# uibk-uncover/ws-unet

Measured on AMD Instinct MI355X. Metric: 512x512 grayscale images/sec (UNet predict), higher is better.
Workload: dtype f16 MFMA on the f16 halves + ONE block-scaled fp4 (e2m1) MFMA per tap pair for both residual cross terms (per-pixel / per-(co, tap) E8M0 scales), fp32 accumulate; planar storage

## Files before the change

### ws_unet_amd/csrc/conv3x3_q.hip

```cpp
#include "wsu_device.h"
#include <cstdlib>

namespace {

constexpr int TW = 32, TH = 16, IW = TW + 2, IH = TH + 2;
constexpr int NPIX = IW * IH;
constexpr int PLANE = NPIX * 16;
constexpr int IN_SEG = (NPIX + 63) / 64;
constexpr int S_LDS = IN_SEG * 256;
constexpr int IN_SLOT = 3 * PLANE + S_LDS;
constexpr int W_GRAN = 9 * 3 * WSU_COB * 16;
constexpr int W_SLOT = W_GRAN + 1024;
constexpr int NIN = 3, NWS = 2;
constexpr int W_BASE = NIN * IN_SLOT;
constexpr int LDS_EXTRA = W_BASE + NWS * W_SLOT;
constexpr int LDS_TOTAL = LDS_EXTRA + 1024 * 4 + 4 * 64 * 4 + 16;
static_assert(LDS_TOTAL <= 160 * 1024 && W_SLOT % 1024 == 0, "LDS budget");
constexpr int NLOAD = 4;
constexpr int W_PIECES = W_SLOT / 1024;
constexpr unsigned OOB = 0xFFFFFFF0u;
constexpr int IN_SLOT_H = 2 * PLANE;
constexpr int W_SLOT_H = 9 * 2 * WSU_COB * 16;
template <int FMT> struct QGeo {
    static_assert(FMT == WSU_PLANAR_Q || FMT == WSU_PLANAR_H, "conv3x3_q_kernel formats: Q and H");
// ... 234 lines not shown
        switch (wv - NWAVE) {
            case 0: q_loader<FMT, 0>(a, smem, lane, lw, G, J); break;
            case 1: q_loader<FMT, 1>(a, smem, lane, lw, G, J); break;
            case 2: q_loader<FMT, 2>(a, smem, lane, lw, G, J); break;
            default: q_loader<FMT, 3>(a, smem, lane, lw, G, J); break;
        }
        return;
    }

    Tile cur = tile_of(a, lw);
    constexpr int MH = MSPLIT ? 1 : 2;
    constexpr bool PIPE = RQ == 4 && !H;
    constexpr bool EPO = !MSPLIT && HC == 0 && RQ != 4;
    f32x16 acc[2][4];
    int kt = 0, j = 0;
    unsigned q_in_off = 0, q_w_off = 0;
    const char* ldsA = smem;
    const char* ldsB = smem;
    int hh_q = hh;
    auto begin_step = [&]() __attribute__((always_inline)) {
        __builtin_amdgcn_s_barrier();
        asm volatile("" ::: "memory");
        q_in_off = (unsigned)(j % NIN) * Gm::in_slot; q_w_off = Gm::w_base + (unsigned)(j % NWS) * Gm::w_slot;
        ldsA = smem + q_w_off + (cur.mh * 32 + l31) * 16;
        ldsB = smem + q_in_off + ((RQ * wv) * IW + l31) * 16;
        hh_q = hh;
        asm volatile("" : "+v"(hh_q));
    };
    auto zero_acc = [&]() __attribute__((always_inline)) {
#pragma unroll
        for (int m = 0; m < MH; ++m)
#pragma unroll
            for (int q = 0; q < RQ; ++q)
#pragma unroll
                for (int r = 0; r < 16; ++r) acc[m][q][r] = 0.f;
    };
    auto main_term = [&](auto tap_c, auto ms_c) __attribute__((always_inline)) {
        constexpr int tap = decltype(tap_c)::value, dy = tap / 3, dx = tap % 3;
        constexpr int ms = decltype(ms_c)::value, ML = ms < 0 ? 0 : ms, MU = ms < 0 ? MH : ms + 1;
        u32x4 ah[2], bh[4];
_Pragma("unroll")
        for (int m = ML; m < MU; ++m) ah[m] = *reinterpret_cast<const u32x4*>(ldsA + ((tap * Gm::w_planes + hh) * 64 + m * 32) * 16);
_Pragma("unroll")
        for (int q = 0; q < RQ; ++q) bh[q] = *reinterpret_cast<const u32x4*>(ldsB + hh * PLANE + ((q + dy) * IW + dx) * 16);
_Pragma("unroll")
        for (int m = ML; m < MU; ++m)
_Pragma("unroll")
            for (int q = 0; q < RQ; ++q) wsu_mfma_f16(ah[m], bh[q], acc[m][q]);
    };
    auto cross_q4 = [&](auto tp_c, auto ms_c) __attribute__((always_inline)) {
        constexpr int tp = decltype(tp_c)::value;
        constexpr int ms = decltype(ms_c)::value, ML = ms < 0 ? 0 : ms, MU = ms < 0 ? MH : ms + 1;
        constexpr int t0 = 2 * tp, t1 = (2 * tp + 1 < 9) ? 2 * tp + 1 : 2 * tp;
        constexpr bool single = 2 * tp + 1 >= 9;
        const int tap = hh_q ? t1 : t0;
        const int pixoff = (tap / 3) * IW + tap % 3;
        u32x4 a4[2], b4[4]; int sa[2], sb[4];
        typedef __attribute__((address_space(3))) const unsigned char lds_cuchar;
        typedef __attribute__((address_space(3))) const int lds_cint;
        typedef __attribute__((address_space(3))) const u32x4 lds_cu32x4;
        lds_char* L = (lds_char*)smem;
        const unsigned wbase = q_w_off + (unsigned)(cur.mh * 32 + l31) * 16u + (unsigned)((tap * 3 + 2) * 64) * 16u;
        const unsigned sabase = q_w_off + W_GRAN + (unsigned)(tap * 64 + cur.mh * 32 + l31);
        const unsigned pix = (unsigned)((RQ * wv) * IW + l31 + pixoff);
_Pragma("unroll")
        for (int m = ML; m < MU; ++m) {
            a4[m] = *(lds_cu32x4*)(L + wbase + m * 32 * 16);
            sa[m] = *(lds_cuchar*)(L + sabase + m * 32);
        }
_Pragma("unroll")
        for (int q = 0; q < RQ; ++q) {
            b4[q] = *(lds_cu32x4*)(L + q_in_off + 2 * PLANE + (pix + q * IW) * 16u);
            sb[q] = *(lds_cint*)(L + q_in_off + 3 * PLANE + (pix + q * IW) * 4u);
        }
        if (single && hh_q) {
            const u32x4 z = mk_u4(0, 0, 0, 0);
_Pragma("unroll")
            for (int m = ML; m < MU; ++m) a4[m] = z;
_Pragma("unroll")
            for (int q = 0; q < RQ; ++q) b4[q] = z;
        }
_Pragma("unroll")
        for (int m = ML; m < MU; ++m)
_Pragma("unroll")
            for (int q = 0; q < RQ; ++q) wsu_mfma_q4(a4[m], b4[q], sa[m], sb[q], acc[m][q]);
    };
    auto units_range = [&](auto ms_c, auto lo_c, auto hi_c) __attribute__((always_inline)) {
        constexpr int lo = decltype(lo_c)::value, hi = decltype(hi_c)::value;
        if constexpr (EPO) asm volatile("" : "+v"(hh_q));
        WSU_STATIC_FOR(hi - lo, i, {
            constexpr int tp = lo + i;
            if constexpr (!H) cross_q4(std::integral_constant<int, tp>{}, ms_c);
            main_term(std::integral_constant<int, 2 * tp>{}, ms_c);
            if constexpr (2 * tp + 1 < 9) main_term(std::integral_constant<int, 2 * tp + 1>{}, ms_c);
        });
    };
    constexpr std::integral_constant<int, -1> all_m{};
    struct Frag { u32x4 a[2]; u32x4 b[4]; int sa[2]; int sb[4]; };
    auto load_unit = [&](auto u_c, Frag& f) __attribute__((always_inline)) {
        constexpr int u = decltype(u_c)::value, tp = u / 3, k = u % 3;
        typedef __attribute__((address_space(3))) const unsigned char lds_cuchar;
        typedef __attribute__((address_space(3))) const int lds_cint;
        typedef __attribute__((address_space(3))) const u32x4 lds_cu32x4;
        lds_char* L = (lds_char*)smem;
        if constexpr (k == 0) {
            constexpr int t0 = 2 * tp, t1 = (2 * tp + 1 < 9) ? 2 * tp + 1 : 2 * tp;
            const int tap = hh_q ? t1 : t0;
            const int pixoff = (tap / 3) * IW + tap % 3;
            const unsigned wbase = q_w_off + (unsigned)(cur.mh * 32 + l31) * 16u + (unsigned)((tap * 3 + 2) * 64) * 16u;
            const unsigned sabase = q_w_off + W_GRAN + (unsigned)(tap * 64 + cur.mh * 32 + l31);
            const unsigned pix = (unsigned)((RQ * wv) * IW + l31 + pixoff);
_Pragma("unroll")
            for (int m = 0; m < MH; ++m) {
                f.a[m] = *(lds_cu32x4*)(L + wbase + m * 32 * 16);
                f.sa[m] = *(lds_cuchar*)(L + sabase + m * 32);
            }
_Pragma("unroll")
            for (int q = 0; q < RQ; ++q) {
                f.b[q] = *(lds_cu32x4*)(L + q_in_off + 2 * PLANE + (pix + q * IW) * 16u);
                f.sb[q] = *(lds_cint*)(L + q_in_off + 3 * PLANE + (pix + q * IW) * 4u);
            }
        } else {
            constexpr int tap = 2 * tp + k - 1, dy = tap / 3, dx = tap % 3;
            const unsigned abase = q_w_off + (unsigned)((cur.mh * 32 + l31) * 16) + (unsigned)(hh_q * 64 * 16);
            const unsigned bbase = q_in_off + (unsigned)(((RQ * wv) * IW + l31) * 16) + (unsigned)(hh_q * PLANE);
_Pragma("unroll")
            for (int m = 0; m < MH; ++m) f.a[m] = *(lds_cu32x4*)(L + abase + ((tap * 3) * 64 + m * 32) * 16);
_Pragma("unroll")
            for (int q = 0; q < RQ; ++q) f.b[q] = *(lds_cu32x4*)(L + bbase + ((q + dy) * IW + dx) * 16);
        }
    };
    auto mma_unit = [&](auto u_c, Frag& f) __attribute__((always_inline)) {
        constexpr int u = decltype(u_c)::value, tp = u / 3, k = u % 3;
        if constexpr (k == 0) {
            if (2 * tp + 1 >= 9 && hh_q) {
                const u32x4 z = mk_u4(0, 0, 0, 0);
_Pragma("unroll")
                for (int m = 0; m < MH; ++m) f.a[m] = z;
_Pragma("unroll")
                for (int q = 0; q < RQ; ++q) f.b[q] = z;
            }
_Pragma("unroll")
            for (int m = 0; m < MH; ++m)
_Pragma("unroll")
                for (int q = 0; q < RQ; ++q) wsu_mfma_q4(f.a[m], f.b[q], f.sa[m], f.sb[q], acc[m][q]);
        } else {
_Pragma("unroll")
            for (int m = 0; m < MH; ++m)
_Pragma("unroll")
                for (int q = 0; q < RQ; ++q) wsu_mfma_f16(f.a[m], f.b[q], acc[m][q]);
        }
    };
    auto units_pipelined = [&]() __attribute__((always_inline)) {
        constexpr int NU = 14;
        Frag fr[2];
        load_unit(std::integral_constant<int, 0>{}, fr[0]);
        WSU_STATIC_FOR(NU, u, {
            if constexpr (u + 1 < NU) load_unit(std::integral_constant<int, u + 1>{}, fr[(u + 1) % 2]);
            __builtin_amdgcn_sched_barrier(0);
            mma_unit(u_c, fr[u % 2]);
            __builtin_amdgcn_sched_barrier(0);
        });
    };
    auto units_all = [&](auto ms_c) __attribute__((always_inline)) {
        if constexpr (PIPE && decltype(ms_c)::value < 0) { units_pipelined(); return; }
        units_range(ms_c, std::integral_constant<int, 0>{}, std::integral_constant<int, 5>{});
    };

    auto finish_tile = [&]() __attribute__((always_inline)) {
        int l31 = l31_k, hh = hh_k;
        asm volatile("" : "+v"(l31), "+v"(hh));
        const int col = cur.x0 + l31;
        const unsigned hw16 = (unsigned)(a.h * a.w) * 16u;
        const int nco = a.cout >> 4;
        float hz[4][HC > 0 ? HC : 1];
        float vmax = 0.f;
        const float relu_floor = a.relu ? 0.f : -__builtin_inff();
#pragma unroll
        for (int q = 0; q < RQ; ++q)
#pragma unroll
            for (int o = 0; o < (HC > 0 ? HC : 1); ++o) hz[q][o] = 0.f;
// ... 26 lines not shown
        };
        auto store_one_a = [&](const f32x4& X, const f32x4& Y, char* base, unsigned plane_bytes, unsigned off, bool ok, bool have) __attribute__((always_inline)) {
            uint32_t xh0, xh1, xlo, yh0, yh1, ylo;
            wsu_split4_f16r8(X, WSU_F8_XLO_DIV, xh0, xh1, xlo);
            wsu_split4_f16r8(Y, WSU_F8_XLO_DIV, yh0, yh1, ylo);
            wsu_swap32(xh0, yh0); wsu_swap32(xh1, yh1);
            uint32_t xlp = xlo, ylp = ylo;
            wsu_swap32(xlo, xlp); wsu_swap32(ylo, ylp);
            const auto rs = __builtin_amdgcn_make_buffer_rsrc(base, 0, have ? (int)(3u * plane_bytes) : 0, 0x00020000);
            __builtin_amdgcn_raw_buffer_store_b128(mk_u4(xh0, xh1, yh0, yh1), rs, (int)(ok ? off + (hh ? plane_bytes : 0u) : OOB), 0, 0);
            __builtin_amdgcn_raw_buffer_store_b128(mk_u4(xlo, xlp, ylo, ylp), rs, (int)((ok && !hh) ? off + 2u * plane_bytes : OOB), 0, 0);
        };
        auto epi_m = [&](auto m_c, auto&& hook) __attribute__((always_inline)) {
            constexpr int m = decltype(m_c)::value;
            constexpr int NH = RQ / 2;
            auto piece = [&](auto cp_c) __attribute__((always_inline)) {
                constexpr int cp = decltype(cp_c)::value;
                const int oc = cur.cb * 4 + (m + cur.mh) * 2 + cp;
                const int co0 = oc * 16 + 4 * hh;
                const bool have_y = a.y != nullptr;
                f32x4 px[2], py[2];
                WSU_STATIC_FOR(RQ / 2, rp, {
                    hook(std::integral_constant<int, NH * cp + rp>{});
                    f32x4 vx[2], vy[2];
                    const f32x4 bx = *reinterpret_cast<const f32x4*>(s_bias + co0), by = *reinterpret_cast<const f32x4*>(s_bias + co0 + 8);
_Pragma("unroll")
                    for (int u = 0; u < 2; ++u) {
_Pragma("unroll")
                        for (int e = 0; e < 4; ++e) {
                            const float x = fmaxf(acc[m][2 * rp + u][8 * cp + e] + bx[e], relu_floor), y = fmaxf(acc[m][2 * rp + u][8 * cp + 4 + e] + by[e], relu_floor);
// ... 47 lines not shown
                    const int gy0 = (cur.y0 >> 1) + (RQ / 2) * wv, gx = (cur.x0 >> 1) + (l31 >> 1);
                    const bool okx = !(l31 & 1) && gx < wp2;
                    const unsigned php16 = (unsigned)(hp * wp2) * 16u;
                    if constexpr (H) {
                        char* base = a.ypool + ((size_t)cur.n * nco + oc) * (2u * php16);
#pragma unroll
                        for (int rp = 0; rp < RQ / 2; ++rp)
                            store_one_h(px[rp], py[rp], base, php16, (unsigned)((gy0 + rp) * wp2 + gx) * 16u, okx && gy0 + rp < hp, true);
                    } else if constexpr (FQ) {
                        const unsigned cbp = (unsigned)wsu_q_chunk_bytes(hp, wp2);
                        const int ptx = (wp2 + 31) >> 5;
                        char* base = a.ypool + ((size_t)cur.n * nco + oc) * cbp;
                        if constexpr (RQ == 4) {
                            store_pair_q(px[0], py[0], px[1], py[1], base, cbp, php16, (unsigned)(gy0 * wp2 + gx) * 16u, (unsigned)((gy0 + 1) * wp2 + gx) * 16u,
                                         wsu_q_soff(gy0, gx, ptx), wsu_q_soff(gy0 + 1, gx, ptx), okx && gy0 < hp, okx && gy0 + 1 < hp, true);
                        } else {
                            store_one_q(px[0], py[0], base, cbp, php16, (unsigned)(gy0 * wp2 + gx) * 16u, wsu_q_soff(gy0, gx, ptx), okx && gy0 < hp, true);
                        }
                    } else {
                        char* base = a.ypool + (((size_t)cur.n * nco + oc) * 3) * php16;
#pragma unroll
                        for (int rp = 0; rp < RQ / 2; ++rp)
                            store_one_a(px[rp], py[rp], base, php16, (unsigned)((gy0 + rp) * wp2 + gx) * 16u, okx && gy0 + rp < hp, true);
                    }
                }
            };
            piece(std::integral_constant<int, 0>{});
            piece(std::integral_constant<int, 1>{});
        };
        auto nothing = [](auto) __attribute__((always_inline)) {};
        if constexpr (EPO) {
            constexpr int NHT = 2 * (RQ / 2);
            epi_m(std::integral_constant<int, 0>{}, [&](auto h_c) __attribute__((always_inline)) {
                constexpr int h = decltype(h_c)::value;
                constexpr int lo = 5 * h / NHT, hi = 5 * (h + 1) / NHT;
                if constexpr (hi > lo) units_range(std::integral_constant<int, 1>{}, std::integral_constant<int, lo>{}, std::integral_constant<int, hi>{});
            });
            epi_m(std::integral_constant<int, 1>{}, nothing);
        } else {
            WSU_STATIC_FOR(MH, m, { (void)m; epi_m(m_c, nothing); });
        }
        if constexpr (HEAD) {
            const size_t hw = (size_t)a.h * a.w;
#pragma unroll
            for (int q = 0; q < RQ; ++q) {
                const int row = cur.y0 + RQ * wv + q;
#pragma unroll
                for (int o = 0; o < HC; ++o)
                    if (o < a.head_cout) {
                        uint32_t mine = __builtin_bit_cast(uint32_t, hz[q][o]), other = mine;
                        wsu_swap32(mine, other);
// ... 1 lines not shown
                        if (!hh && row < a.h && col < a.w) {
                            const size_t plane = ((size_t)cur.n * a.head_cout + o) * hw;
                            const uint32_t off = (uint32_t)(row * a.w + col);
                            if (a.head_logit) (a.head_logit + plane)[off] = z;
                            (a.head_out + plane)[off] = 1.f / (1.f + expf(-z));
                        }
                    }
            }
        }
        if (a.range_flag && (a.y || POOL) && __builtin_amdgcn_ballot_w64(!(vmax <= (H ? WSU_F16_RANGE : WSU_F8_RANGE))) != 0 && lane == 0)
            atomicOr(a.range_flag, 1u);
        ++kt;
        if (j + 1 < J) cur = tile_of(a, lw + kt * G);
    };
    for (int t = 0; t < K; ++t) {
        zero_acc();
        for (int cc = 1; cc < a.nch; ++cc) { begin_step(); units_all(all_m); ++j; }
        begin_step();
        if constexpr (EPO) units_all(std::integral_constant<int, 0>{});
        else units_all(all_m);
        __builtin_amdgcn_sched_barrier(0);
        finish_tile();
        ++j;
    }
}

__global__ void pack_conv3x3_f4_kernel(const float* __restrict__ w, char* __restrict__ dst, int cin, int cout) {
    const int nch = cin / 16;
    const long long total = (long long)(cout / WSU_COB) * nch * 9 * WSU_COB;
    for (long long d = (long long)blockIdx.x * blockDim.x + threadIdx.x; d < total; d += (long long)gridDim.x * blockDim.x) {
        long long t = d;
        const int co = (int)(t % WSU_COB); t /= WSU_COB;
        const int tap = (int)(t % 9); t /= 9;
        const int c = (int)(t % nch); const int cb = (int)(t / nch);
        float v[16], r[16];
// ... 274 lines not shown
```

### ws_unet_amd/csrc/conv3x3_qu.hip

```cpp
#include "wsu_device.h"

namespace {

constexpr int TW = 32, TH = 16;
constexpr int CW = 17, CH = 9, CPIX = CW * CH;
constexpr int NPIX_S = 4 * CPIX;
constexpr int PLANE_S = NPIX_S * 16;
constexpr int SEG_S = (NPIX_S + 63) / 64;
constexpr int IN_S = 3 * PLANE_S + SEG_S * 256;
constexpr int LP = 33, LH = TH / 2 + 2, LW_ = TW / 2 + 2;
constexpr int NPIX_L = LP * LH;
constexpr int PLANE_L = NPIX_L * 16;
constexpr int SEG_L = (NPIX_L + 63) / 64;
constexpr int IN_L = 3 * PLANE_L + SEG_L * 256;
constexpr int W_GRAN_S = 9 * 3 * WSU_COB * 16;
constexpr int W_S = W_GRAN_S + 1024;
constexpr int W_UNITS_L = 8;
constexpr int W_GRAN_L = W_UNITS_L * 3 * WSU_COB * 16;
constexpr int W_L = W_GRAN_L + 1024;
constexpr int PIECES_S = W_S / 1024, PIECES_L = W_L / 1024;
constexpr int REGION = 80640;
constexpr int OFF_SW = IN_S, OFF_LIN = W_L, OFF_LW1 = W_L + IN_L;
constexpr int LDS_BIAS = 2 * REGION;
constexpr int MAX_COUT = 512;
// ... 195 lines not shown
    const int cls = wv & 3, py = cls >> 1, px = cls & 1, rh = wv >> 2;
    const int l31 = lane & 31, hh = lane >> 5;
    const int lrow = l31 >> 4, lcol = lrow ? ((l31 + 15) & 15) : l31;
    const unsigned laneS = (unsigned)(((4 * rh + lrow) * CW + lcol) * 16), laneL = (unsigned)(((4 * rh + lrow) * LP + lcol) * 16);
    constexpr unsigned QS = 2 * CW * 16, QL = 2 * LP * 16;
    Tile cur = tile_of(a, lw);
    f32x16 acc[2][2];
    unsigned region = 0;
    unsigned in_off = 0, w_off = 0;
    auto next_region = [&]() __attribute__((always_inline)) { const unsigned r = region; region ^= (unsigned)REGION; return r; };
    int hh_q = hh;
    typedef __attribute__((address_space(3))) const unsigned char lds_cuchar;
    typedef __attribute__((address_space(3))) const int lds_cint;
    typedef __attribute__((address_space(3))) const u32x4 lds_cu32x4;
    lds_char* L = (lds_char*)smem;
    auto sync_step = [&]() __attribute__((always_inline)) {
        __builtin_amdgcn_s_barrier();
        asm volatile("" ::: "memory");
        hh_q = hh;
        asm volatile("" : "+v"(hh_q));
    };
    auto tap_s = [&](int ky, int kx) __attribute__((always_inline)) {
        return (unsigned)(((((py + ky) & 1) * 2 + ((px + kx) & 1)) * CPIX + ((py + ky) >> 1) * CW + ((px + kx) >> 1)) * 16);
    };
    auto skip_units = [&]() __attribute__((always_inline)) {
        WSU_STATIC_FOR(5, tp, {
            constexpr int t0 = 2 * tp, t1 = (2 * tp + 1 < 9) ? 2 * tp + 1 : 2 * tp;
            if constexpr (!H) {
                const unsigned tapo = hh_q ? tap_s(t1 / 3, t1 % 3) : tap_s(t0 / 3, t0 % 3);
                const int tap = hh_q ? t1 : t0;
                u32x4 a4[2], b4[2]; int sa[2], sb[2];
                const unsigned wb = w_off + (unsigned)((tap * 3 + 2) * 64 + l31) * 16u, sab = w_off + W_GRAN_S + (unsigned)(tap * 64 + l31);
                const unsigned pb = tapo + laneS;
_Pragma("unroll")
                for (int m = 0; m < 2; ++m) { a4[m] = *(lds_cu32x4*)(L + wb + m * 512); sa[m] = *(lds_cuchar*)(L + sab + m * 32); }
_Pragma("unroll")
                for (int q = 0; q < 2; ++q) {
                    b4[q] = *(lds_cu32x4*)(L + in_off + 2 * PLANE_S + pb + q * QS);
                    sb[q] = *(lds_cint*)(L + in_off + 3 * PLANE_S + ((pb + q * QS) >> 2));
                }
                if (2 * tp + 1 >= 9 && hh_q) {
                    const u32x4 z = mk_u4(0, 0, 0, 0);
                    a4[0] = z; a4[1] = z; b4[0] = z; b4[1] = z;
                }
_Pragma("unroll")
                for (int m = 0; m < 2; ++m)
_Pragma("unroll")
                    for (int q = 0; q < 2; ++q) wsu_mfma_q4(a4[m], b4[q], sa[m], sb[q], acc[m][q]);
            }
            WSU_STATIC_FOR((2 * tp + 1 < 9 ? 2 : 1), k, {
                constexpr int tap = 2 * tp + k;
                u32x4 ah[2], bh[2];
                const unsigned wb = w_off + (unsigned)((tap * WPL) * 64 + l31) * 16u + (unsigned)hh * 1024u;
                const unsigned pb = in_off + (unsigned)hh * PLANE_S + tap_s(tap / 3, tap % 3) + laneS;
_Pragma("unroll")
                for (int m = 0; m < 2; ++m) ah[m] = *(lds_cu32x4*)(L + wb + m * 512);
_Pragma("unroll")
                for (int q = 0; q < 2; ++q) bh[q] = *(lds_cu32x4*)(L + pb + q * QS);
_Pragma("unroll")
                for (int m = 0; m < 2; ++m)
_Pragma("unroll")
                    for (int q = 0; q < 2; ++q) wsu_mfma_f16(ah[m], bh[q], acc[m][q]);
            });
        });
    };
    auto low_units = [&](int dy) __attribute__((always_inline)) {
        const unsigned rowo = (unsigned)(((py + dy) * LP + px) * 16);
        if constexpr (!H) {
            const int u = cls * 2 + hh_q;
            u32x4 a4[2], b4[2]; int sa[2], sb[2];
            const unsigned wb = w_off + (unsigned)((u * 3 + 2) * 64 + l31) * 16u, sab = w_off + W_GRAN_L + (unsigned)(u * 64 + l31);
            const unsigned pb = rowo + (unsigned)hh_q * 16u + laneL;
_Pragma("unroll")
            for (int m = 0; m < 2; ++m) { a4[m] = *(lds_cu32x4*)(L + wb + m * 512); sa[m] = *(lds_cuchar*)(L + sab + m * 32); }
_Pragma("unroll")
            for (int q = 0; q < 2; ++q) {
                b4[q] = *(lds_cu32x4*)(L + in_off + 2 * PLANE_L + pb + q * QL);
                sb[q] = *(lds_cint*)(L + in_off + 3 * PLANE_L + ((pb + q * QL) >> 2));
            }
_Pragma("unroll")
            for (int m = 0; m < 2; ++m)
_Pragma("unroll")
                for (int q = 0; q < 2; ++q) wsu_mfma_q4(a4[m], b4[q], sa[m], sb[q], acc[m][q]);
        }
        WSU_STATIC_FOR(2, dx, {
            u32x4 ah[2], bh[2];
            const unsigned wb = w_off + (unsigned)(((cls * 2 + dx) * WPL) * 64 + l31) * 16u + (unsigned)hh * 1024u;
            const unsigned pb = in_off + (unsigned)hh * PLANE_L + rowo + dx * 16u + laneL;
_Pragma("unroll")
            for (int m = 0; m < 2; ++m) ah[m] = *(lds_cu32x4*)(L + wb + m * 512);
_Pragma("unroll")
            for (int q = 0; q < 2; ++q) bh[q] = *(lds_cu32x4*)(L + pb + q * QL);
_Pragma("unroll")
            for (int m = 0; m < 2; ++m)
_Pragma("unroll")
                for (int q = 0; q < 2; ++q) wsu_mfma_f16(ah[m], bh[q], acc[m][q]);
        });
    };

    auto finish_tile = [&]() __attribute__((always_inline)) {
        int l31o = l31, hho = hh, lro = lrow, lco = lcol;
        asm volatile("" : "+v"(l31o), "+v"(hho), "+v"(lro), "+v"(lco));
        const unsigned hw16 = (unsigned)(a.h * a.w) * 16u;
        const unsigned cbytes = (unsigned)wsu_q_chunk_bytes(a.h, a.w);
        const int nco = a.cout >> 4;
        const int X = cur.x0 + 2 * lco + px;
        const int Y0 = cur.y0 + 2 * (4 * rh + lro) + py, Y1 = Y0 + 4;
// ... 30 lines not shown
                const u32x4 qg = wsu_q4_pair(dh0, dr0, dh1, dr1);
                char* base = a.y + ((size_t)cur.n * nco + oc) * cbytes;
                const auto rs = __builtin_amdgcn_make_buffer_rsrc(base, 0, (int)cbytes, 0x00020000);
                const unsigned hp = hho ? hw16 : 0u;
                __builtin_amdgcn_raw_buffer_store_b128(g0, rs, (int)(ok0 ? off0 + hp : OOB), 0, 0);
                __builtin_amdgcn_raw_buffer_store_b128(g1, rs, (int)(ok1 ? off1 + hp : OOB), 0, 0);
                const bool okm = hho ? ok1 : ok0;
                __builtin_amdgcn_raw_buffer_store_b128(qg, rs, (int)(okm ? (hho ? off1 : off0) + 2u * hw16 : OOB), 0, 0);
                __builtin_amdgcn_raw_buffer_store_b8((unsigned char)(hho ? sb1 : sb0), rs, (int)(okm ? 3u * hw16 + (hho ? so1 : so0) : OOB), 0, 0);
            });
        });
        if (a.range_flag && __builtin_amdgcn_ballot_w64(!(vmax <= (H ? WSU_F16_RANGE : WSU_F8_RANGE))) != 0 && lane == 0) atomicOr(a.range_flag, 1u);
    };

    for (int t = 0; t < K; ++t) {
#pragma unroll
        for (int m = 0; m < 2; ++m)
#pragma unroll
            for (int q = 0; q < 2; ++q)
#pragma unroll
                for (int r = 0; r < 16; ++r) acc[m][q][r] = 0.f;
        for (int c = 0; c < a.nchS; ++c) {
            sync_step();
            const unsigned r = next_region();
            in_off = r; w_off = r + OFF_SW;
            skip_units();
        }
        for (int c = 0; c < a.nchL; ++c) {
            sync_step();
            const unsigned r = next_region();
            in_off = r + OFF_LIN;
            w_off = r;
            low_units(0);
            w_off = r + OFF_LW1;
            low_units(1);
        }
        finish_tile();
        if (t + 1 < K) cur = tile_of(a, lw + (t + 1) * G);
    }
}

template <int FMT>
__global__ void pack_up_low_kernel(const float* __restrict__ w3, const float* __restrict__ wt, char* __restrict__ dst, float* __restrict__ wc_dense,
                                   int cup, int c2, int cl, int cout) {
    const int nchL = cl / 16, ctot = cup + c2;
    const long long total = (long long)(cout / WSU_COB) * nchL * 2 * W_UNITS_L * WSU_COB;
    for (long long d = (long long)blockIdx.x * blockDim.x + threadIdx.x; d < total; d += (long long)gridDim.x * blockDim.x) {
        long long t = d;
        const int co = (int)(t % WSU_COB); t /= WSU_COB;
        const int u = (int)(t % W_UNITS_L); t /= W_UNITS_L;
// ... 166 lines not shown
```

### ws_unet_amd/csrc/wsu_device.h

```cpp
#pragma once
#include <hip/hip_runtime.h>
#include <stdint.h>
#include <type_traits>
#include "../../include/wsu.h"

typedef __attribute__((ext_vector_type(8))) __bf16 bf16x8;
typedef __attribute__((ext_vector_type(16))) float f32x16;
typedef __attribute__((ext_vector_type(4))) float f32x4;
typedef __attribute__((ext_vector_type(4))) uint32_t u32x4;
typedef __attribute__((ext_vector_type(2))) uint32_t u32x2;
__host__ __device__ __forceinline__ u32x4 mk_u4(uint32_t a, uint32_t b, uint32_t c, uint32_t d) { u32x4 v = {a, b, c, d}; return v; }
__host__ __device__ __forceinline__ u32x2 mk_u2(uint32_t a, uint32_t b) { u32x2 v = {a, b}; return v; }
__host__ __device__ __forceinline__ f32x4 mk_f4(float a, float b, float c, float d) { f32x4 v = {a, b, c, d}; return v; }

void wsu_set_error(const char* fmt, ...);
int wsu_check_launch(const char* what);
#define WSU_REQUIRE(cond, ...)            \
    do {                                  \
        if (!(cond)) {                    \
            wsu_set_error(__VA_ARGS__);   \
            return WSU_ERR_ARG;           \
        }                                 \
    } while (0)
#define WSU_INTERNAL extern "C" __attribute__((visibility("hidden")))
// ... 214 lines not shown
    const int e = wsu_q4_block_exp(wsu_f16x16_max_abs_bits(h0, h1));
    const float sc = wsu_pow2f(e), scr = wsu_pow2f(e - 11);
    sb = (uint32_t)(e + 127);
    uint32_t q2 = 0, q3 = 0;
    q2 = __builtin_amdgcn_cvt_scalef32_pk_fp4_f32(q2, r[0], r[1], scr, 0); q2 = __builtin_amdgcn_cvt_scalef32_pk_fp4_f32(q2, r[2], r[3], scr, 1);
    q2 = __builtin_amdgcn_cvt_scalef32_pk_fp4_f32(q2, r[4], r[5], scr, 2); q2 = __builtin_amdgcn_cvt_scalef32_pk_fp4_f32(q2, r[6], r[7], scr, 3);
    q3 = __builtin_amdgcn_cvt_scalef32_pk_fp4_f32(q3, r[8], r[9], scr, 0); q3 = __builtin_amdgcn_cvt_scalef32_pk_fp4_f32(q3, r[10], r[11], scr, 1);
    q3 = __builtin_amdgcn_cvt_scalef32_pk_fp4_f32(q3, r[12], r[13], scr, 2); q3 = __builtin_amdgcn_cvt_scalef32_pk_fp4_f32(q3, r[14], r[15], scr, 3);
    q = mk_u4(wsu_f16x8_to_fp4(h0, sc), wsu_f16x8_to_fp4(h1, sc), q2, q3);
}
__device__ __forceinline__ void wsu_mfma_q4(const u32x4& a, const u32x4& b, int scale_a, int scale_b, f32x16& acc) {
    const i32x8 av = {(int)a.x, (int)a.y, (int)a.z, (int)a.w, 0, 0, 0, 0}, bv = {(int)b.x, (int)b.y, (int)b.z, (int)b.w, 0, 0, 0, 0};
    acc = __builtin_amdgcn_mfma_scale_f32_32x32x64_f8f6f4(av, bv, acc, 4, 4, 0, scale_a, 0, scale_b);
}

__device__ __forceinline__ u32x2 wsu_f16x8_to_fp8_grad(const u32x4& h) {
    const _Float16 m = (_Float16)112.f;
    const f16x8 lim = {m, m, m, m, m, m, m, m};
    const f16x8 c = __builtin_elementwise_max(__builtin_elementwise_min(__builtin_bit_cast(f16x8, h), lim), -lim);
    i16x2 lo = {0, 0}, hi = {0, 0};
    lo = __builtin_amdgcn_cvt_scalef32_pk_fp8_f16(lo, __builtin_shufflevector(c, c, 0, 1), WSU_F8_G_DIV, false);
    lo = __builtin_amdgcn_cvt_scalef32_pk_fp8_f16(lo, __builtin_shufflevector(c, c, 2, 3), WSU_F8_G_DIV, true);
    hi = __builtin_amdgcn_cvt_scalef32_pk_fp8_f16(hi, __builtin_shufflevector(c, c, 4, 5), WSU_F8_G_DIV, false);
    hi = __builtin_amdgcn_cvt_scalef32_pk_fp8_f16(hi, __builtin_shufflevector(c, c, 6, 7), WSU_F8_G_DIV, true);
    return mk_u2(__builtin_bit_cast(uint32_t, lo), __builtin_bit_cast(uint32_t, hi));
}
__device__ __forceinline__ void wsu_mfma_f16(const u32x4& a, const u32x4& b, f32x16& acc) {
    acc = __builtin_amdgcn_mfma_f32_32x32x16_f16(__builtin_bit_cast(f16x8, a), __builtin_bit_cast(f16x8, b), acc, 0, 0, 0);
}
__device__ __forceinline__ void wsu_mfma_f8x2(const u32x4& a_blk0, const u32x4& a_blk1, const u32x4& b_blk0, const u32x4& b_blk1,
                                              int scale_a, int scale_b, f32x16& acc) {
    i32x8 a = {(int)a_blk0.x, (int)a_blk0.y, (int)a_blk0.z, (int)a_blk0.w, (int)a_blk1.x, (int)a_blk1.y, (int)a_blk1.z, (int)a_blk1.w};
    i32x8 b = {(int)b_blk0.x, (int)b_blk0.y, (int)b_blk0.z, (int)b_blk0.w, (int)b_blk1.x, (int)b_blk1.y, (int)b_blk1.z, (int)b_blk1.w};
    acc = __builtin_amdgcn_mfma_scale_f32_32x32x64_f8f6f4(a, b, acc, 0, 0, 0, scale_a, 0, scale_b);
}

__device__ __forceinline__ float wsu_bf16_to_f32(uint16_t v) { return __builtin_bit_cast(float, (uint32_t)v << 16); }

template <int MODE>
__device__ __forceinline__ void wsu_mfma_step(const u32x4& a, const u32x4& b, f32x16& acc) {
    if constexpr (MODE == WSU_MODE_F32) {
        const f32x4 af = __builtin_bit_cast(f32x4, a), bf = __builtin_bit_cast(f32x4, b);
        acc = __builtin_amdgcn_mfma_f32_32x32x2f32(af[0], bf[0], acc, 0, 0, 0);
// ... 23 lines not shown
```

Baseline: 3703.

## Precompute LDS addresses before barrier and fold accumulator zeroing into first MFMA

Computes LDS slot offsets incrementally and hoists per-step base addresses (including the first tap-pair cross-term addresses) ahead of the workgroup barrier, so address arithmetic overlaps the barrier wait instead of following it. The first MFMA of each tile now uses a zero-accumulator variant, which removes the explicit zeroing of the accumulator registers. In the odd-RQ epilogue, two single-channel stores are paired across lanes into one wider store. This adds code complexity and more live VGPRs for the precomputed addresses, which may raise register pressure.

After: 3788 (median of 6 runs). +2.3%, better.

```diff
diff --git a/ws_unet_amd/csrc/conv3x3_q.hip b/ws_unet_amd/csrc/conv3x3_q.hip
--- a/ws_unet_amd/csrc/conv3x3_q.hip
+++ b/ws_unet_amd/csrc/conv3x3_q.hip
@@ -272,18 +272,38 @@
     constexpr bool EPO = !MSPLIT && HC == 0 && RQ != 4;
     f32x16 acc[2][4];
     int kt = 0, j = 0;
-    unsigned q_in_off = 0, q_w_off = 0;
-    const char* ldsA = smem;
-    const char* ldsB = smem;
+    unsigned q_in_off = 0, q_w_off = Gm::w_base;
+    unsigned nx_in = 0, nx_w = Gm::w_base;
+    unsigned a_off = 0, b_off = 0, hd_w = 0, hd_sa = 0, hd_b = 0, hd_sb = 0;
     int hh_q = hh;
+    typedef __attribute__((address_space(3))) const unsigned char lds_cuchar;
+    typedef __attribute__((address_space(3))) const int lds_cint;
+    typedef __attribute__((address_space(3))) const u32x4 lds_cu32x4;
+    lds_char* const L = (lds_char*)smem;
+    const unsigned Lb = (unsigned)(size_t)L;
+    auto at = [](unsigned addr) __attribute__((always_inline)) { return (lds_char*)(size_t)addr; };
     auto begin_step = [&]() __attribute__((always_inline)) {
+        q_in_off = nx_in; q_w_off = nx_w;
+        nx_in = nx_in + (unsigned)Gm::in_slot == (unsigned)(NIN * Gm::in_slot) ? 0u : nx_in + (unsigned)Gm::in_slot;
+        static_assert(NWS == 2, "nx_w toggles between the two weight slots the loaders fill as s % NWS");
+        nx_w = (unsigned)(2 * Gm::w_base + Gm::w_slot) - nx_w;
+        hh_q = hh;
+        asm volatile("" : "+v"(hh_q));
+        a_off = Lb + q_w_off + (unsigned)((cur.mh * 32 + l31) * 16) + (unsigned)(hh * 64 * 16);
+        b_off = Lb + q_in_off + (unsigned)(((RQ * wv) * IW + l31) * 16) + (unsigned)(hh * PLANE);
+        if constexpr (!H) {
+            const int tap = hh_q ? 1 : 0;
+            const unsigned pix = (unsigned)((RQ * wv) * IW + l31 + tap);
+            hd_w = Lb + q_w_off + (unsigned)(cur.mh * 32 + l31) * 16u + (unsigned)((tap * 3 + 2) * 64) * 16u;
+            hd_sa = Lb + q_w_off + W_GRAN + (unsigned)(tap * 64 + cur.mh * 32 + l31);
+            hd_b = Lb + q_in_off + 2 * PLANE + pix * 16u;
+            hd_sb = Lb + q_in_off + 3 * PLANE + pix * 4u;
+            asm volatile("" : "+v"(a_off), "+v"(b_off), "+v"(hd_w), "+v"(hd_sa), "+v"(hd_b), "+v"(hd_sb));
+        } else {
+            asm volatile("" : "+v"(a_off), "+v"(b_off));
+        }
         __builtin_amdgcn_s_barrier();
         asm volatile("" ::: "memory");
-        q_in_off = (unsigned)(j % NIN) * Gm::in_slot; q_w_off = Gm::w_base + (unsigned)(j % NWS) * Gm::w_slot;
-        ldsA = smem + q_w_off + (cur.mh * 32 + l31) * 16;
-        ldsB = smem + q_in_off + ((RQ * wv) * IW + l31) * 16;
-        hh_q = hh;
-        asm volatile("" : "+v"(hh_q));
     };
     auto zero_acc = [&]() __attribute__((always_inline)) {
 #pragma unroll
@@ -293,43 +313,47 @@
 #pragma unroll
                 for (int r = 0; r < 16; ++r) acc[m][q][r] = 0.f;
     };
-    auto main_term = [&](auto tap_c, auto ms_c) __attribute__((always_inline)) {
+    auto main_term = [&](auto tap_c, auto ms_c, auto first_c) __attribute__((always_inline)) {
         constexpr int tap = decltype(tap_c)::value, dy = tap / 3, dx = tap % 3;
         constexpr int ms = decltype(ms_c)::value, ML = ms < 0 ? 0 : ms, MU = ms < 0 ? MH : ms + 1;
+        constexpr bool FIRST = decltype(first_c)::value;
         u32x4 ah[2], bh[4];
 _Pragma("unroll")
-        for (int m = ML; m < MU; ++m) ah[m] = *reinterpret_cast<const u32x4*>(ldsA + ((tap * Gm::w_planes + hh) * 64 + m * 32) * 16);
-_Pragma("unroll")
-        for (int q = 0; q < RQ; ++q) bh[q] = *reinterpret_cast<const u32x4*>(ldsB + hh * PLANE + ((q + dy) * IW + dx) * 16);
+        for (int m = ML; m < MU; ++m) ah[m] = *(lds_cu32x4*)(at(a_off) + ((tap * Gm::w_planes) * 64 + m * 32) * 16);
+_Pragma("unroll")
+        for (int q = 0; q < RQ; ++q) bh[q] = *(lds_cu32x4*)(at(b_off) + ((q + dy) * IW + dx) * 16);
 _Pragma("unroll")
         for (int m = ML; m < MU; ++m)
 _Pragma("unroll")
-            for (int q = 0; q < RQ; ++q) wsu_mfma_f16(ah[m], bh[q], acc[m][q]);
-    };
-    auto cross_q4 = [&](auto tp_c, auto ms_c) __attribute__((always_inline)) {
+            for (int q = 0; q < RQ; ++q) {
+                if constexpr (FIRST) acc[m][q] = wsu_mfma_f16_z(ah[m], bh[q]);
+                else wsu_mfma_f16(ah[m], bh[q], acc[m][q]);
+            }
+    };
+    auto cross_q4 = [&](auto tp_c, auto ms_c, auto first_c) __attribute__((always_inline)) {
         constexpr int tp = decltype(tp_c)::value;
         constexpr int ms = decltype(ms_c)::value, ML = ms < 0 ? 0 : ms, MU = ms < 0 ? MH : ms + 1;
+        constexpr bool FIRST = decltype(first_c)::value;
         constexpr int t0 = 2 * tp, t1 = (2 * tp + 1 < 9) ? 2 * tp + 1 : 2 * tp;
         constexpr bool single = 2 * tp + 1 >= 9;
+        constexpr bool HEAD_UNIT = tp == 0 && ms <= 0;
         const int tap = hh_q ? t1 : t0;
         const int pixoff = (tap / 3) * IW + tap % 3;
         u32x4 a4[2], b4[4]; int sa[2], sb[4];
-        typedef __attribute__((address_space(3))) const unsigned char lds_cuchar;
-        typedef __attribute__((address_space(3))) const int lds_cint;
-        typedef __attribute__((address_space(3))) const u32x4 lds_cu32x4;
-        lds_char* L = (lds_char*)smem;
-        const unsigned wbase = q_w_off + (unsigned)(cur.mh * 32 + l31) * 16u + (unsigned)((tap * 3 + 2) * 64) * 16u;
-        const unsigned sabase = q_w_off + W_GRAN + (unsigned)(tap * 64 + cur.mh * 32 + l31);
         const unsigned pix = (unsigned)((RQ * wv) * IW + l31 + pixoff);
+        const unsigned wbase = HEAD_UNIT ? hd_w : Lb + q_w_off + (unsigned)(cur.mh * 32 + l31) * 16u + (unsigned)((tap * 3 + 2) * 64) * 16u;
+        const unsigned sabase = HEAD_UNIT ? hd_sa : Lb + q_w_off + W_GRAN + (unsigned)(tap * 64 + cur.mh * 32 + l31);
+        const unsigned bbase = HEAD_UNIT ? hd_b : Lb + q_in_off + 2 * PLANE + pix * 16u;
+        const unsigned sbbase = HEAD_UNIT ? hd_sb : Lb + q_in_off + 3 * PLANE + pix * 4u;
 _Pragma("unroll")
         for (int m = ML; m < MU; ++m) {
-            a4[m] = *(lds_cu32x4*)(L + wbase + m * 32 * 16);
-            sa[m] = *(lds_cuchar*)(L + sabase + m * 32);
+            a4[m] = *(lds_cu32x4*)(at(wbase) + m * 32 * 16);
+            sa[m] = *(lds_cuchar*)(at(sabase) + m * 32);
         }
 _Pragma("unroll")
         for (int q = 0; q < RQ; ++q) {
-            b4[q] = *(lds_cu32x4*)(L + q_in_off + 2 * PLANE + (pix + q * IW) * 16u);
-            sb[q] = *(lds_cint*)(L + q_in_off + 3 * PLANE + (pix + q * IW) * 4u);
+            b4[q] = *(lds_cu32x4*)(at(bbase) + (q * IW) * 16u);
+            sb[q] = *(lds_cint*)(at(sbbase) + (q * IW) * 4u);
         }
         if (single && hh_q) {
             const u32x4 z = mk_u4(0, 0, 0, 0);
@@ -341,42 +365,47 @@
 _Pragma("unroll")
         for (int m = ML; m < MU; ++m)
 _Pragma("unroll")
-            for (int q = 0; q < RQ; ++q) wsu_mfma_q4(a4[m], b4[q], sa[m], sb[q], acc[m][q]);
-    };
-    auto units_range = [&](auto ms_c, auto lo_c, auto hi_c) __attribute__((always_inline)) {
+            for (int q = 0; q < RQ; ++q) {
+                if constexpr (FIRST) acc[m][q] = wsu_mfma_q4_z(a4[m], b4[q], sa[m], sb[q]);
+                else wsu_mfma_q4(a4[m], b4[q], sa[m], sb[q], acc[m][q]);
+            }
+    };
+    constexpr std::false_type not_first{};
+    constexpr std::true_type tile_first{};
+    auto units_range = [&](auto ms_c, auto lo_c, auto hi_c, auto first_c) __attribute__((always_inline)) {
         constexpr int lo = decltype(lo_c)::value, hi = decltype(hi_c)::value;
-        if constexpr (EPO) asm volatile("" : "+v"(hh_q));
+        constexpr bool FIRST = decltype(first_c)::value;
+        static_assert(!FIRST || lo == 0, "a tile opens with tap pair 0");
+        if constexpr (EPO && !(lo == 0 && decltype(ms_c)::value <= 0)) asm volatile("" : "+v"(hh_q));
         WSU_STATIC_FOR(hi - lo, i, {
             constexpr int tp = lo + i;
-            if constexpr (!H) cross_q4(std::integral_constant<int, tp>{}, ms_c);
-            main_term(std::integral_constant<int, 2 * tp>{}, ms_c);
-            if constexpr (2 * tp + 1 < 9) main_term(std::integral_constant<int, 2 * tp + 1>{}, ms_c);
+            if constexpr (!H) cross_q4(std::integral_constant<int, tp>{}, ms_c, std::integral_constant<bool, FIRST && tp == 0>{});
+            main_term(std::integral_constant<int, 2 * tp>{}, ms_c, std::integral_constant<bool, FIRST && H && tp == 0>{});
+            if constexpr (2 * tp + 1 < 9) main_term(std::integral_constant<int, 2 * tp + 1>{}, ms_c, not_first);
         });
     };
     constexpr std::integral_constant<int, -1> all_m{};
     struct Frag { u32x4 a[2]; u32x4 b[4]; int sa[2]; int sb[4]; };
     auto load_unit = [&](auto u_c, Frag& f) __attribute__((always_inline)) {
         constexpr int u = decltype(u_c)::value, tp = u / 3, k = u % 3;
-        typedef __attribute__((address_space(3))) const unsigned char lds_cuchar;
-        typedef __attribute__((address_space(3))) const int lds_cint;
-        typedef __attribute__((address_space(3))) const u32x4 lds_cu32x4;
-        lds_char* L = (lds_char*)smem;
         if constexpr (k == 0) {
             constexpr int t0 = 2 * tp, t1 = (2 * tp + 1 < 9) ? 2 * tp + 1 : 2 * tp;
             const int tap = hh_q ? t1 : t0;
             const int pixoff = (tap / 3) * IW + tap % 3;
-            const unsigned wbase = q_w_off + (unsigned)(cur.mh * 32 + l31) * 16u + (unsigned)((tap * 3 + 2) * 64) * 16u;
-            const unsigned sabase = q_w_off + W_GRAN + (unsigned)(tap * 64 + cur.mh * 32 + l31);
             const unsigned pix = (unsigned)((RQ * wv) * IW + l31 + pixoff);
+            const unsigned wbase = u == 0 ? hd_w : Lb + q_w_off + (unsigned)(cur.mh * 32 + l31) * 16u + (unsigned)((tap * 3 + 2) * 64) * 16u;
+            const unsigned sabase = u == 0 ? hd_sa : Lb + q_w_off + W_GRAN + (unsigned)(tap * 64 + cur.mh * 32 + l31);
+            const unsigned bbase = u == 0 ? hd_b : Lb + q_in_off + 2 * PLANE + pix * 16u;
+            const unsigned sbbase = u == 0 ? hd_sb : Lb + q_in_off + 3 * PLANE + pix * 4u;
 _Pragma("unroll")
             for (int m = 0; m < MH; ++m) {
-                f.a[m] = *(lds_cu32x4*)(L + wbase + m * 32 * 16);
-                f.sa[m] = *(lds_cuchar*)(L + sabase + m * 32);
+                f.a[m] = *(lds_cu32x4*)(at(wbase) + m * 32 * 16);
+                f.sa[m] = *(lds_cuchar*)(at(sabase) + m * 32);
             }
 _Pragma("unroll")
             for (int q = 0; q < RQ; ++q) {
-                f.b[q] = *(lds_cu32x4*)(L + q_in_off + 2 * PLANE + (pix + q * IW) * 16u);
-                f.sb[q] = *(lds_cint*)(L + q_in_off + 3 * PLANE + (pix + q * IW) * 4u);
+                f.b[q] = *(lds_cu32x4*)(at(bbase) + (q * IW) * 16u);
+                f.sb[q] = *(lds_cint*)(at(sbbase) + (q * IW) * 4u);
             }
         } else {
             constexpr int tap = 2 * tp + k - 1, dy = tap / 3, dx = tap % 3;
@@ -388,8 +417,9 @@
             for (int q = 0; q < RQ; ++q) f.b[q] = *(lds_cu32x4*)(L + bbase + ((q + dy) * IW + dx) * 16);
         }
     };
-    auto mma_unit = [&](auto u_c, Frag& f) __attribute__((always_inline)) {
+    auto mma_unit = [&](auto u_c, Frag& f, auto first_c) __attribute__((always_inline)) {
         constexpr int u = decltype(u_c)::value, tp = u / 3, k = u % 3;
+        constexpr bool FIRST = decltype(first_c)::value && u == 0;
         if constexpr (k == 0) {
             if (2 * tp + 1 >= 9 && hh_q) {
                 const u32x4 z = mk_u4(0, 0, 0, 0);
@@ -401,7 +431,10 @@
 _Pragma("unroll")
             for (int m = 0; m < MH; ++m)
 _Pragma("unroll")
-                for (int q = 0; q < RQ; ++q) wsu_mfma_q4(f.a[m], f.b[q], f.sa[m], f.sb[q], acc[m][q]);
+                for (int q = 0; q < RQ; ++q) {
+                    if constexpr (FIRST) acc[m][q] = wsu_mfma_q4_z(f.a[m], f.b[q], f.sa[m], f.sb[q]);
+                    else wsu_mfma_q4(f.a[m], f.b[q], f.sa[m], f.sb[q], acc[m][q]);
+                }
         } else {
 _Pragma("unroll")
             for (int m = 0; m < MH; ++m)
@@ -409,20 +442,20 @@
                 for (int q = 0; q < RQ; ++q) wsu_mfma_f16(f.a[m], f.b[q], acc[m][q]);
         }
     };
-    auto units_pipelined = [&]() __attribute__((always_inline)) {
+    auto units_pipelined = [&](auto first_c) __attribute__((always_inline)) {
         constexpr int NU = 14;
         Frag fr[2];
         load_unit(std::integral_constant<int, 0>{}, fr[0]);
         WSU_STATIC_FOR(NU, u, {
             if constexpr (u + 1 < NU) load_unit(std::integral_constant<int, u + 1>{}, fr[(u + 1) % 2]);
             __builtin_amdgcn_sched_barrier(0);
-            mma_unit(u_c, fr[u % 2]);
+            mma_unit(u_c, fr[u % 2], first_c);
             __builtin_amdgcn_sched_barrier(0);
         });
     };
-    auto units_all = [&](auto ms_c) __attribute__((always_inline)) {
-        if constexpr (PIPE && decltype(ms_c)::value < 0) { units_pipelined(); return; }
-        units_range(ms_c, std::integral_constant<int, 0>{}, std::integral_constant<int, 5>{});
+    auto units_all = [&](auto ms_c, auto first_c) __attribute__((always_inline)) {
+        if constexpr (PIPE && decltype(ms_c)::value < 0) { units_pipelined(first_c); return; }
+        units_range(ms_c, std::integral_constant<int, 0>{}, std::integral_constant<int, 5>{}, first_c);
     };
 
     auto finish_tile = [&]() __attribute__((always_inline)) {
@@ -479,6 +512,7 @@
         auto epi_m = [&](auto m_c, auto&& hook) __attribute__((always_inline)) {
             constexpr int m = decltype(m_c)::value;
             constexpr int NH = RQ / 2;
+            f32x4 spx, spy;
             auto piece = [&](auto cp_c) __attribute__((always_inline)) {
                 constexpr int cp = decltype(cp_c)::value;
                 const int oc = cur.cb * 4 + (m + cur.mh) * 2 + cp;
@@ -556,8 +590,16 @@
                         if constexpr (RQ == 4) {
                             store_pair_q(px[0], py[0], px[1], py[1], base, cbp, php16, (unsigned)(gy0 * wp2 + gx) * 16u, (unsigned)((gy0 + 1) * wp2 + gx) * 16u,
                                          wsu_q_soff(gy0, gx, ptx), wsu_q_soff(gy0 + 1, gx, ptx), okx && gy0 < hp, okx && gy0 + 1 < hp, true);
+                        } else if constexpr (cp == 0) {
+                            spx = px[0]; spy = py[0];
                         } else {
-                            store_one_q(px[0], py[0], base, cbp, php16, (unsigned)(gy0 * wp2 + gx) * 16u, wsu_q_soff(gy0, gx, ptx), okx && gy0 < hp, true);
+                            static_assert(cp == 1, "piece 1 closes the pair: its chunk follows piece 0's");
+                            const bool odd = (l31 & 1) != 0;
+                            f32x4 sx, sy;
+_Pragma("unroll")
+                            for (int e = 0; e < 4; ++e) { sx[e] = odd ? px[0][e] : spx[e]; sy[e] = odd ? py[0][e] : spy[e]; }
+                            const unsigned coff = odd ? cbp : 0u;
+                            store_one_q(sx, sy, base - cbp, 2u * cbp, php16, (unsigned)(gy0 * wp2 + gx) * 16u + coff, wsu_q_soff(gy0, gx, ptx) + coff, gx < wp2 && gy0 < hp, true);
                         }
                     } else {
                         char* base = a.ypool + (((size_t)cur.n * nco + oc) * 3) * php16;
@@ -576,7 +618,7 @@
             epi_m(std::integral_constant<int, 0>{}, [&](auto h_c) __attribute__((always_inline)) {
                 constexpr int h = decltype(h_c)::value;
                 constexpr int lo = 5 * h / NHT, hi = 5 * (h + 1) / NHT;
-                if constexpr (hi > lo) units_range(std::integral_constant<int, 1>{}, std::integral_constant<int, lo>{}, std::integral_constant<int, hi>{});
+                if constexpr (hi > lo) units_range(std::integral_constant<int, 1>{}, std::integral_constant<int, lo>{}, std::integral_constant<int, hi>{}, not_first);
             });
             epi_m(std::integral_constant<int, 1>{}, nothing);
         } else {
@@ -608,11 +650,15 @@
         if (j + 1 < J) cur = tile_of(a, lw + kt * G);
     };
     for (int t = 0; t < K; ++t) {
-        zero_acc();
-        for (int cc = 1; cc < a.nch; ++cc) { begin_step(); units_all(all_m); ++j; }
+        if (a.nch == 1) {
+            zero_acc();
+        } else {
+            begin_step(); units_all(all_m, tile_first); ++j;
+            for (int cc = 2; cc < a.nch; ++cc) { begin_step(); units_all(all_m, not_first); ++j; }
+        }
         begin_step();
-        if constexpr (EPO) units_all(std::integral_constant<int, 0>{});
-        else units_all(all_m);
+        if constexpr (EPO) units_all(std::integral_constant<int, 0>{}, not_first);
+        else units_all(all_m, not_first);
         __builtin_amdgcn_sched_barrier(0);
         finish_tile();
         ++j;
diff --git a/ws_unet_amd/csrc/conv3x3_qu.hip b/ws_unet_amd/csrc/conv3x3_qu.hip
--- a/ws_unet_amd/csrc/conv3x3_qu.hip
+++ b/ws_unet_amd/csrc/conv3x3_qu.hip
@@ -233,30 +233,54 @@
     typedef __attribute__((address_space(3))) const int lds_cint;
     typedef __attribute__((address_space(3))) const u32x4 lds_cu32x4;
     lds_char* L = (lds_char*)smem;
-    auto sync_step = [&]() __attribute__((always_inline)) {
+    const unsigned Lb = (unsigned)(size_t)L;
+    auto at = [](unsigned addr) __attribute__((always_inline)) { return (lds_char*)(size_t)addr; };
+    auto tap_s = [&](int ky, int kx) __attribute__((always_inline)) {
+        return (unsigned)(((((py + ky) & 1) * 2 + ((px + kx) & 1)) * CPIX + ((py + ky) >> 1) * CW + ((px + kx) >> 1)) * 16);
+    };
+    unsigned a_off = 0, b_off = 0, hd_w = 0, hd_sa = 0, hd_b = 0, hd_sb = 0;
+    auto sync_step = [&](auto low_c) __attribute__((always_inline)) {
+        constexpr bool LOW = decltype(low_c)::value;
+        const unsigned r = next_region();
+        in_off = LOW ? r + OFF_LIN : r;
+        w_off = LOW ? r : r + OFF_SW;
+        hh_q = hh;
+        asm volatile("" : "+v"(hh_q));
+        a_off = Lb + w_off + (unsigned)l31 * 16u + (unsigned)hh * 1024u;
+        b_off = Lb + in_off + (unsigned)hh * (LOW ? PLANE_L : PLANE_S) + (LOW ? laneL : laneS);
+        if constexpr (!H) {
+            const int u = LOW ? cls * 2 + hh_q : hh_q;
+            const unsigned pb = LOW ? (unsigned)((py * LP + px) * 16) + (unsigned)hh_q * 16u + laneL : (hh_q ? tap_s(0, 1) : tap_s(0, 0)) + laneS;
+            hd_w = Lb + w_off + (unsigned)((u * 3 + 2) * 64 + l31) * 16u;
+            hd_sa = Lb + w_off + (LOW ? W_GRAN_L : W_GRAN_S) + (unsigned)(u * 64 + l31);
+            hd_b = Lb + in_off + 2 * (LOW ? PLANE_L : PLANE_S) + pb;
+            hd_sb = Lb + in_off + 3 * (LOW ? PLANE_L : PLANE_S) + (pb >> 2);
+            asm volatile("" : "+v"(a_off), "+v"(b_off), "+v"(hd_w), "+v"(hd_sa), "+v"(hd_b), "+v"(hd_sb));
+        } else {
+            asm volatile("" : "+v"(a_off), "+v"(b_off));
+        }
         __builtin_amdgcn_s_barrier();
         asm volatile("" ::: "memory");
-        hh_q = hh;
-        asm volatile("" : "+v"(hh_q));
-    };
-    auto tap_s = [&](int ky, int kx) __attribute__((always_inline)) {
-        return (unsigned)(((((py + ky) & 1) * 2 + ((px + kx) & 1)) * CPIX + ((py + ky) >> 1) * CW + ((px + kx) >> 1)) * 16);
-    };
-    auto skip_units = [&]() __attribute__((always_inline)) {
+    };
+    auto skip_units = [&](auto first_c) __attribute__((always_inline)) {
+        constexpr bool FIRST = decltype(first_c)::value;
         WSU_STATIC_FOR(5, tp, {
             constexpr int t0 = 2 * tp, t1 = (2 * tp + 1 < 9) ? 2 * tp + 1 : 2 * tp;
             if constexpr (!H) {
                 const unsigned tapo = hh_q ? tap_s(t1 / 3, t1 % 3) : tap_s(t0 / 3, t0 % 3);
                 const int tap = hh_q ? t1 : t0;
                 u32x4 a4[2], b4[2]; int sa[2], sb[2];
-                const unsigned wb = w_off + (unsigned)((tap * 3 + 2) * 64 + l31) * 16u, sab = w_off + W_GRAN_S + (unsigned)(tap * 64 + l31);
                 const unsigned pb = tapo + laneS;
-_Pragma("unroll")
-                for (int m = 0; m < 2; ++m) { a4[m] = *(lds_cu32x4*)(L + wb + m * 512); sa[m] = *(lds_cuchar*)(L + sab + m * 32); }
+                const unsigned wb = tp == 0 ? hd_w : Lb + w_off + (unsigned)((tap * 3 + 2) * 64 + l31) * 16u;
+                const unsigned sab = tp == 0 ? hd_sa : Lb + w_off + W_GRAN_S + (unsigned)(tap * 64 + l31);
+                const unsigned bb = tp == 0 ? hd_b : Lb + in_off + 2 * PLANE_S + pb;
+                const unsigned sbb = tp == 0 ? hd_sb : Lb + in_off + 3 * PLANE_S + (pb >> 2);
+_Pragma("unroll")
+                for (int m = 0; m < 2; ++m) { a4[m] = *(lds_cu32x4*)(at(wb) + m * 512); sa[m] = *(lds_cuchar*)(at(sab) + m * 32); }
 _Pragma("unroll")
                 for (int q = 0; q < 2; ++q) {
-                    b4[q] = *(lds_cu32x4*)(L + in_off + 2 * PLANE_S + pb + q * QS);
-                    sb[q] = *(lds_cint*)(L + in_off + 3 * PLANE_S + ((pb + q * QS) >> 2));
+                    b4[q] = *(lds_cu32x4*)(at(bb) + q * QS);
+                    sb[q] = *(lds_cint*)(at(sbb) + q * (QS >> 2));
                 }
                 if (2 * tp + 1 >= 9 && hh_q) {
                     const u32x4 z = mk_u4(0, 0, 0, 0);
@@ -265,37 +289,47 @@
 _Pragma("unroll")
                 for (int m = 0; m < 2; ++m)
 _Pragma("unroll")
-                    for (int q = 0; q < 2; ++q) wsu_mfma_q4(a4[m], b4[q], sa[m], sb[q], acc[m][q]);
+                    for (int q = 0; q < 2; ++q) {
+                        if constexpr (FIRST && tp == 0) acc[m][q] = wsu_mfma_q4_z(a4[m], b4[q], sa[m], sb[q]);
+                        else wsu_mfma_q4(a4[m], b4[q], sa[m], sb[q], acc[m][q]);
+                    }
             }
             WSU_STATIC_FOR((2 * tp + 1 < 9 ? 2 : 1), k, {
                 constexpr int tap = 2 * tp + k;
                 u32x4 ah[2], bh[2];
-                const unsigned wb = w_off + (unsigned)((tap * WPL) * 64 + l31) * 16u + (unsigned)hh * 1024u;
-                const unsigned pb = in_off + (unsigned)hh * PLANE_S + tap_s(tap / 3, tap % 3) + laneS;
-_Pragma("unroll")
-                for (int m = 0; m < 2; ++m) ah[m] = *(lds_cu32x4*)(L + wb + m * 512);
-_Pragma("unroll")
-                for (int q = 0; q < 2; ++q) bh[q] = *(lds_cu32x4*)(L + pb + q * QS);
+                const unsigned pb = b_off + tap_s(tap / 3, tap % 3);
+_Pragma("unroll")
+                for (int m = 0; m < 2; ++m) ah[m] = *(lds_cu32x4*)(at(a_off) + ((tap * WPL) * 64) * 16 + m * 512);
+_Pragma("unroll")
+                for (int q = 0; q < 2; ++q) bh[q] = *(lds_cu32x4*)(at(pb) + q * QS);
 _Pragma("unroll")
                 for (int m = 0; m < 2; ++m)
 _Pragma("unroll")
-                    for (int q = 0; q < 2; ++q) wsu_mfma_f16(ah[m], bh[q], acc[m][q]);
+                    for (int q = 0; q < 2; ++q) {
+                        if constexpr (FIRST && H && tap == 0) acc[m][q] = wsu_mfma_f16_z(ah[m], bh[q]);
+                        else wsu_mfma_f16(ah[m], bh[q], acc[m][q]);
+                    }
             });
         });
     };
-    auto low_units = [&](int dy) __attribute__((always_inline)) {
+    auto low_units = [&](auto dy_c) __attribute__((always_inline)) {
+        constexpr int dy = decltype(dy_c)::value;
+        constexpr unsigned WDY = dy ? (unsigned)(OFF_LW1) : 0u;
         const unsigned rowo = (unsigned)(((py + dy) * LP + px) * 16);
         if constexpr (!H) {
             const int u = cls * 2 + hh_q;
             u32x4 a4[2], b4[2]; int sa[2], sb[2];
-            const unsigned wb = w_off + (unsigned)((u * 3 + 2) * 64 + l31) * 16u, sab = w_off + W_GRAN_L + (unsigned)(u * 64 + l31);
             const unsigned pb = rowo + (unsigned)hh_q * 16u + laneL;
-_Pragma("unroll")
-            for (int m = 0; m < 2; ++m) { a4[m] = *(lds_cu32x4*)(L + wb + m * 512); sa[m] = *(lds_cuchar*)(L + sab + m * 32); }
+            const unsigned wb = dy == 0 ? hd_w : Lb + w_off + WDY + (unsigned)((u * 3 + 2) * 64 + l31) * 16u;
+            const unsigned sab = dy == 0 ? hd_sa : Lb + w_off + WDY + W_GRAN_L + (unsigned)(u * 64 + l31);
+            const unsigned bb = dy == 0 ? hd_b : Lb + in_off + 2 * PLANE_L + pb;
+            const unsigned sbb = dy == 0 ? hd_sb : Lb + in_off + 3 * PLANE_L + (pb >> 2);
+_Pragma("unroll")
+            for (int m = 0; m < 2; ++m) { a4[m] = *(lds_cu32x4*)(at(wb) + m * 512); sa[m] = *(lds_cuchar*)(at(sab) + m * 32); }
 _Pragma("unroll")
             for (int q = 0; q < 2; ++q) {
-                b4[q] = *(lds_cu32x4*)(L + in_off + 2 * PLANE_L + pb + q * QL);
-                sb[q] = *(lds_cint*)(L + in_off + 3 * PLANE_L + ((pb + q * QL) >> 2));
+                b4[q] = *(lds_cu32x4*)(at(bb) + q * QL);
+                sb[q] = *(lds_cint*)(at(sbb) + q * (QL >> 2));
             }
 _Pragma("unroll")
             for (int m = 0; m < 2; ++m)
@@ -304,12 +338,12 @@
         }
         WSU_STATIC_FOR(2, dx, {
             u32x4 ah[2], bh[2];
-            const unsigned wb = w_off + (unsigned)(((cls * 2 + dx) * WPL) * 64 + l31) * 16u + (unsigned)hh * 1024u;
-            const unsigned pb = in_off + (unsigned)hh * PLANE_L + rowo + dx * 16u + laneL;
-_Pragma("unroll")
-            for (int m = 0; m < 2; ++m) ah[m] = *(lds_cu32x4*)(L + wb + m * 512);
-_Pragma("unroll")
-            for (int q = 0; q < 2; ++q) bh[q] = *(lds_cu32x4*)(L + pb + q * QL);
+            const unsigned wb = a_off + WDY + (unsigned)(((cls * 2 + dx) * WPL) * 64) * 16u;
+            const unsigned pb = b_off + rowo + dx * 16u;
+_Pragma("unroll")
+            for (int m = 0; m < 2; ++m) ah[m] = *(lds_cu32x4*)(at(wb) + m * 512);
+_Pragma("unroll")
+            for (int q = 0; q < 2; ++q) bh[q] = *(lds_cu32x4*)(at(pb) + q * QL);
 _Pragma("unroll")
             for (int m = 0; m < 2; ++m)
 _Pragma("unroll")
@@ -370,26 +404,16 @@
     };
 
     for (int t = 0; t < K; ++t) {
-#pragma unroll
-        for (int m = 0; m < 2; ++m)
-#pragma unroll
-            for (int q = 0; q < 2; ++q)
-#pragma unroll
-                for (int r = 0; r < 16; ++r) acc[m][q][r] = 0.f;
-        for (int c = 0; c < a.nchS; ++c) {
-            sync_step();
-            const unsigned r = next_region();
-            in_off = r; w_off = r + OFF_SW;
-            skip_units();
+        sync_step(std::false_type{});
+        skip_units(std::true_type{});
+        for (int c = 1; c < a.nchS; ++c) {
+            sync_step(std::false_type{});
+            skip_units(std::false_type{});
         }
         for (int c = 0; c < a.nchL; ++c) {
-            sync_step();
-            const unsigned r = next_region();
-            in_off = r + OFF_LIN;
-            w_off = r;
-            low_units(0);
-            w_off = r + OFF_LW1;
-            low_units(1);
+            sync_step(std::true_type{});
+            low_units(std::integral_constant<int, 0>{});
+            low_units(std::integral_constant<int, 1>{});
         }
         finish_tile();
         if (t + 1 < K) cur = tile_of(a, lw + (t + 1) * G);
diff --git a/ws_unet_amd/csrc/wsu_device.h b/ws_unet_amd/csrc/wsu_device.h
--- a/ws_unet_amd/csrc/wsu_device.h
+++ b/ws_unet_amd/csrc/wsu_device.h
@@ -252,6 +252,12 @@
     acc = __builtin_amdgcn_mfma_scale_f32_32x32x64_f8f6f4(av, bv, acc, 4, 4, 0, scale_a, 0, scale_b);
 }
 
+__device__ __forceinline__ f32x16 wsu_mfma_q4_z(const u32x4& a, const u32x4& b, int scale_a, int scale_b) {
+    const i32x8 av = {(int)a.x, (int)a.y, (int)a.z, (int)a.w, 0, 0, 0, 0}, bv = {(int)b.x, (int)b.y, (int)b.z, (int)b.w, 0, 0, 0, 0};
+    const f32x16 z = {0.f, 0.f, 0.f, 0.f, 0.f, 0.f, 0.f, 0.f, 0.f, 0.f, 0.f, 0.f, 0.f, 0.f, 0.f, 0.f};
+    return __builtin_amdgcn_mfma_scale_f32_32x32x64_f8f6f4(av, bv, z, 4, 4, 0, scale_a, 0, scale_b);
+}
+
 __device__ __forceinline__ u32x2 wsu_f16x8_to_fp8_grad(const u32x4& h) {
     const _Float16 m = (_Float16)112.f;
     const f16x8 lim = {m, m, m, m, m, m, m, m};
@@ -265,6 +271,10 @@
 }
 __device__ __forceinline__ void wsu_mfma_f16(const u32x4& a, const u32x4& b, f32x16& acc) {
     acc = __builtin_amdgcn_mfma_f32_32x32x16_f16(__builtin_bit_cast(f16x8, a), __builtin_bit_cast(f16x8, b), acc, 0, 0, 0);
+}
+__device__ __forceinline__ f32x16 wsu_mfma_f16_z(const u32x4& a, const u32x4& b) {
+    const f32x16 z = {0.f, 0.f, 0.f, 0.f, 0.f, 0.f, 0.f, 0.f, 0.f, 0.f, 0.f, 0.f, 0.f, 0.f, 0.f, 0.f};
+    return __builtin_amdgcn_mfma_f32_32x32x16_f16(__builtin_bit_cast(f16x8, a), __builtin_bit_cast(f16x8, b), z, 0, 0, 0);
 }
 __device__ __forceinline__ void wsu_mfma_f8x2(const u32x4& a_blk0, const u32x4& a_blk1, const u32x4& b_blk0, const u32x4& b_blk1,
                                               int scale_a, int scale_b, f32x16& acc) {
```
